# nunofachada/cl_ops

Hardware: AMD Instinct MI355X
Metric: Mkeys/s sorting 2^28 uint32 (satradix, 4-bit digits); achieved % of HBM roofline (higher is better)
Workload: dtype u32

## Files before the change

### cl_ops_amd/_hip.py

```python
import ctypes as C
import os

_HERE = os.path.dirname(os.path.abspath(__file__))
LIB_PATH = os.environ.get("CLO_HIP_LIBRARY") or os.path.join(_HERE, "lib", "libcl_ops_hip.so")

if not os.path.exists(LIB_PATH):
    raise ImportError(
        "cl_ops_amd: %s is missing. Build it with `python -c 'import __graft_entry__ as g; g.build()'` "
        "or `make -C cl_ops_amd/csrc` (needs hipcc). There is no fallback path." % LIB_PATH)

lib = C.CDLL(LIB_PATH, mode=C.RTLD_GLOBAL)

vp, sz, ci = C.c_void_p, C.c_size_t, C.c_int


class DeviceProps(C.Structure):
    _fields_ = [("name", C.c_char * 128), ("compute_units", ci), ("max_threads_per_block", ci),
                ("wavefront_size", ci), ("lds_bytes_per_block", sz), ("global_mem_bytes", sz),
                ("gcn_arch", C.c_char * 64)]


def _sig(name, restype, *argtypes):
    try:
        f = getattr(lib, name)
# ... 23 lines not shown
_sig("clo_hip_host_register", ci, vp, sz)
_sig("clo_hip_host_unregister", ci, vp)
_sig("clo_hip_stream_is_capturing", ci, vp)
_sig("clo_hip_graph_capture_begin", ci, vp)
_sig("clo_hip_graph_capture_end", ci, vp, C.POINTER(vp))
_sig("clo_hip_graph_launch", ci, vp, vp)
_sig("clo_hip_graph_destroy", ci, vp)
_sig("clo_hip_timing_enabled", ci)
_sig("clo_hip_event_create", ci, C.POINTER(vp))
_sig("clo_hip_event_destroy", ci, vp)
_sig("clo_hip_event_record", ci, vp, vp)
_sig("clo_hip_event_synchronize", ci, vp)
_sig("clo_hip_event_query", ci, vp)
_sig("clo_hip_env_refresh", None)
_sig("clo_hip_event_elapsed_ms", ci, vp, vp, C.POINTER(C.c_float))
_sig("clo_hip_stream_wait_event", ci, vp, vp)
_sig("clo_hip_error_string", C.c_char_p, ci)
_sig("clo_hip_scan_workspace_bytes", sz, sz, ci, ci)
_sig("clo_hip_scan_workspace_init", ci, vp, sz, vp)
_sig("clo_hip_scan_workspace_forget", ci, vp)
_sig("clo_hip_scan_workspace_set_epoch", ci, vp, C.c_uint, vp)
_sig("clo_hip_scan_exclusive", ci, vp, vp, sz, ci, ci, ci, vp, sz, vp)
_sig("clo_hip_scan_exclusive_carry", ci, vp, vp, sz, ci, ci, ci, vp, vp, vp, sz, vp)
_sig("clo_hip_scan_fp_workspace_bytes", sz, sz, ci)
_sig("clo_hip_scan_is_typed", ci, ci, ci)
_sig("clo_hip_scan_typed_workspace_bytes", sz, sz, ci)
_sig("clo_hip_scan_exclusive_typed", ci, vp, vp, sz, ci, ci, vp, sz, vp)
_sig("clo_hip_scan_exclusive_fp", ci, vp, vp, sz, ci, ci, vp, sz, vp)
_sig("clo_hip_reduce_sum", ci, vp, sz, ci, ci, vp, vp)
_sig("clo_hip_radix_workspace_bytes", sz, sz, ci, ci, ci)
_sig("clo_hip_radix_polls", ci, sz, ci, ci)
_sig("clo_hip_radix_sort", ci, vp, vp, vp, sz, ci, ci, ci, ci, ci, vp, sz, vp)
_sig("clo_hip_radix_takes_first_digits", ci, sz, ci, ci, ci)
_sig("clo_hip_radix_sort_fed", ci, vp, vp, vp, sz, ci, ci, ci, ci, ci, vp, vp, sz, vp)
_sig("clo_hip_radix_seg_workspace_bytes", sz, sz, ci, ci, ci)
_sig("clo_hip_radix_sort_segmented", ci, vp, vp, vp, sz, C.POINTER(sz), ci, C.POINTER(sz), C.POINTER(sz), C.POINTER(ci), ci,
     ci, ci, ci, ci, vp, sz, vp, C.POINTER(ci))
_sig("clo_hip_radix_sort_segmented2", ci, vp, vp, vp, vp, sz, C.POINTER(sz), ci, C.POINTER(sz), C.POINTER(sz), C.POINTER(ci), C.POINTER(ci), ci,
     ci, ci, ci, ci, vp, sz, vp, C.POINTER(ci))
_sig("clo_hip_msd_histogram", ci, vp, sz, ci, ci, ci, ci, vp, vp)
_sig("clo_hip_msd_partition", ci, vp, vp, sz, ci, ci, ci, ci, vp, vp, sz, vp)
_sig("clo_hip_msd_workspace_bytes", sz, sz, ci, ci)
_sig("clo_hip_bitonic_padded_numel", sz, sz)
_sig("clo_hip_bitonic_simple", ci, vp, sz, ci, ci, ci, ci, ci, ci, C.POINTER(ci), vp)
_sig("clo_hip_bitonic_tiled", ci, vp, sz, ci, ci, ci, ci, ci, ci, C.POINTER(ci), vp)
_sig("clo_hip_bitonic_any", ci, vp, sz, ci, ci, ci, ci, ci, ci, C.POINTER(ci), vp)
_sig("clo_hip_kernel_lds_bytes", sz, C.c_char_p, ci, ci)
_sig("clo_hip_bitonic_jit_create", ci, ci, ci, C.c_char_p, C.c_char_p, C.c_char_p, C.POINTER(vp), C.POINTER(C.c_char_p))
_sig("clo_hip_bitonic_jit_destroy", None, vp)
_sig("clo_hip_bitonic_jit_sort", ci, vp, vp, sz, ci, C.POINTER(ci), vp)
_sig("clo_hip_bitonic_jit_gselect", ci, vp, vp, vp, sz, vp)
_sig("clo_hip_check_status", ci, vp, vp)
_sig("clo_hip_rccl_unique_id", ci, vp)
_sig("clo_hip_rccl_comm_create", ci, C.POINTER(vp), vp, ci, ci)
_sig("clo_hip_rccl_comm_destroy", ci, vp)
_sig("clo_hip_rccl_comm_abort", ci, vp)
_sig("clo_hip_rccl_all_gather_u64", ci, vp, vp, vp, sz, vp)
_sig("clo_hip_rccl_all_to_all_v", ci, vp, ci, ci, vp, vp, vp, vp, vp, vp, vp)
_sig("clo_hip_set_launch_observer", ci, vp, vp)
_sig("clo_hip_radix_jit_create", ci, ci, ci, C.c_char_p, C.c_char_p, C.POINTER(vp), C.POINTER(C.c_char_p))
_sig("clo_hip_radix_jit_destroy", None, vp)
_sig("clo_hip_radix_jit_sort", ci, vp, vp, vp, vp, vp, sz, ci, vp, sz, vp)
_sig("clo_hip_timing_enable", ci, ci)
_sig("clo_hip_timing_reset", ci)
_sig("clo_hip_timing_read", ci, C.c_char_p, C.POINTER(C.c_uint), C.POINTER(C.c_float))

# ... 27 lines not shown
```

### cl_ops_amd/csrc/hip/clo_hip_internal.h

```cpp
#ifndef CLO_HIP_INTERNAL_H
#define CLO_HIP_INTERNAL_H

#include <stddef.h>
#include <stdint.h>

#include "clo_hip.h"

#define CLO_WS_STATUS_OFFSET 0
#define CLO_WS_EPOCH_WORD    2
#define CLO_WS_DONE_WORD     3
#define CLO_WS_TICKET_WORD   16
#define CLO_WS_MAX_PASSES    64
#define CLO_WS_HEADER_BYTES  512

struct clo_hip_env_t { unsigned max_spins; int radix_sweep; int r1_pools; int no_digits; int bitonic_merge2; };
const clo_hip_env_t* clo_hip_env();
int clo_radixw_preload();

inline bool clo_misaligned(const void* p, size_t align) { return ((uintptr_t) p & (align - 1)) != 0; }
inline bool clo_ws_misaligned(const void* ws) { return clo_misaligned(ws, CLO_HIP_WORKSPACE_ALIGN); }

#ifdef __HIPCC__
#include <hip/hip_runtime.h>

void clo_timing_begin(const char* label, hipStream_t s);
void clo_timing_end(hipStream_t s);
struct clo_timing_scope {
	hipStream_t s;
	clo_timing_scope(const char* label, hipStream_t stream) : s(stream) { clo_timing_begin(label, s); }
	~clo_timing_scope() { clo_timing_end(s); }
};

struct clo_keyx {
	unsigned long long sign, field;
	int kind;
};
template <typename E>
__device__ __forceinline__ E clo_keyx_fwd(E x, const clo_keyx& k) {
	if (k.kind == 1) return (E) (x ^ (E) k.sign);
	if (k.kind == 2) return (E) (x ^ ((x & (E) k.sign) ? (E) k.field : (E) k.sign));
	return x;
}
template <typename E>
__device__ __forceinline__ E clo_keyx_inv(E x, const clo_keyx& k) {
	if (k.kind == 1) return (E) (x ^ (E) k.sign);
	if (k.kind == 2) return (E) (x ^ ((x & (E) k.sign) ? (E) k.sign : (E) k.field));
	return x;
}
inline clo_keyx clo_keyx_make(int kind, int key_shift, int key_bits) {
	clo_keyx k = { 0, 0, 0 };
	if (kind == 1 || kind == 2) {
		k.kind = kind;
		k.sign = 1ull << (key_shift + key_bits - 1);
		k.field = (key_bits >= 64 ? ~0ull : ((1ull << key_bits) - 1ull)) << key_shift;
	}
	return k;
}

struct clo_kv_io {
	const void* keys_in;
	const unsigned* values_in;
	void* keys_out;
	unsigned* values_out;
};

size_t clo_radix4_workspace_bytes(size_t n, int elem_size, int digit_bits, int key_bits);
int clo_radix4_sort_kv(const clo_kv_io& io, void* pairs_a, void* pairs_b, size_t n, int key_size, int key_shift,
	int key_bits, int digit_bits, clo_keyx kx, void* ws, hipStream_t s);
size_t clo_radix4_partition_workspace_bytes(size_t n, int elem_size, int bits);
int clo_radix4_partition(const void* src, void* dst, size_t n, int elem_size, unsigned shift, int bits,
	unsigned long long* counts, void* ws, hipStream_t s);
int clo_radix4_sort(const void* src, void* dst, void* tmp, size_t n, int elem_size, int key_shift,
	int key_bits, int digit_bits, clo_keyx kx, const unsigned char* first_dig, void* ws, hipStream_t s);
int clo_radix4_takes_first_digits(size_t n, int elem_size, int digit_bits);
size_t clo_radix4_lds_bytes(int elem_size, int digit_bits);
int clo_radix1_applies(size_t n, int elem_size, int digit_bits);
size_t clo_radix1_workspace_bytes(size_t n, int elem_size, int key_bits);
int clo_radix1_sort(const void* src, void* dst, void* tmp, size_t n, int elem_size, int key_shift, int key_bits,
	clo_keyx kx, void* ws, unsigned* status, hipStream_t s);
int clo_bitonic_tiled_e1(void* data, size_t numel, int key_shift, int key_bits, int key_size, int key_kind, int descending, int* launches, hipStream_t s);
int clo_bitonic_tiled_e2(void* data, size_t numel, int key_shift, int key_bits, int key_size, int key_kind, int descending, int* launches, hipStream_t s);
int clo_bitonic_tiled_e4(void* data, size_t numel, int key_shift, int key_bits, int key_size, int key_kind, int descending, int* launches, hipStream_t s);
int clo_bitonic_tiled_e8(void* data, size_t numel, int key_shift, int key_bits, int key_size, int key_kind, int descending, int* launches, hipStream_t s);
size_t clo_radixw_lds_bytes(int digit_bits);
struct clo_radix_counters { unsigned* thist; unsigned* toff; unsigned* partial; unsigned* tinfo; unsigned tiles; bool big; };
int clo_radixw_launch_tilehist(const void* in, size_t n, int elem_size, int bits, unsigned shift, unsigned mask,
	const clo_radix_counters& c, clo_keyx kx, hipStream_t s);
int clo_radixw_launch_tilehist_kv(const void* keys, size_t n, int key_size, int bits, unsigned shift, unsigned mask,
	const clo_radix_counters& c, clo_keyx kx, hipStream_t s);
int clo_radixw_launch_tilehist_bytes(const unsigned char* dig, size_t n, int elem_size, int bits, unsigned mask,
	const clo_radix_counters& c, hipStream_t s);
int clo_radixw_launch_offsets(int bits, const clo_radix_counters& c, const unsigned** dbase, hipStream_t s);
size_t clo_radixw_partial_rows(size_t tiles);

#define CLO_SEG_MAX 256
struct clo_seg_tile { unsigned in_base, count_seg, out_base, seg_n; };
struct clo_seg_chunk { unsigned t0, tend, c_first, seg_last; };
struct clo_seg_pieces {
	unsigned n[CLO_SEG_MAX], in_base[CLO_SEG_MAX];
	unsigned short seg[CLO_SEG_MAX];
};
struct clo_seg_tables { const clo_seg_tile* tiles; const clo_seg_chunk* chunks; unsigned ntiles, nchunks, nseg; };
int clo_radixw_launch_tilehist_seg(const void* in, const void* in2, const clo_seg_tables& sg, int elem_size, int bits, unsigned shift, unsigned mask,
	const clo_radix_counters& c, hipStream_t s);
int clo_radixw_launch_tilehist_bytes_seg(const unsigned char* dig, const clo_seg_tables& sg, int elem_size, int bits, unsigned mask,
	const clo_radix_counters& c, hipStream_t s);
int clo_radixw_launch_offsets_seg(int bits, const clo_radix_counters& c, const clo_seg_tables& sg, const unsigned** dbase, hipStream_t s);
// ... 86 lines not shown
```

### cl_ops_amd/csrc/hip/clo_hip_radix.hip

```cpp
#include <hip/hip_runtime.h>

#include "clo_hip.h"
#include "clo_hip_internal.h"

namespace {

constexpr int HIST_THREADS = 256;
constexpr int HIST_ITEMS = 16;

template <typename E>
__global__ __launch_bounds__(HIST_THREADS)
void clo_msd_hist_kernel(const E* __restrict__ in, size_t n, unsigned shift, unsigned mask,
	unsigned long long* __restrict__ counts) {
	__shared__ unsigned h[HIST_THREADS / 64][8];
	const unsigned tid = threadIdx.x, wave = tid >> 6;
	if (tid < (HIST_THREADS / 64) * 8) (&h[0][0])[tid] = 0;
	__syncthreads();
	const size_t chunk = (size_t) HIST_THREADS * HIST_ITEMS;
	for (size_t base = (size_t) blockIdx.x * chunk; base < n; base += (size_t) gridDim.x * chunk) {
		#pragma unroll
		for (int i = 0; i < HIST_ITEMS; ++i) {
			const size_t idx = base + (size_t) i * HIST_THREADS + tid;
			if (idx < n) atomicAdd(&h[wave][(unsigned) (in[idx] >> shift) & mask & 7u], 1u);
		}
// ... 3 lines not shown
		unsigned s = 0;
		#pragma unroll
		for (int w = 0; w < HIST_THREADS / 64; ++w) s += h[w][tid];
		if (s) atomicAdd(&counts[tid], (unsigned long long) s);
	}
}

template <typename E>
int msd_hist_impl(const void* src, size_t n, unsigned shift, unsigned mask, uint64_t* counts, hipStream_t s) {
	unsigned blocks = (unsigned) ((n + HIST_THREADS * HIST_ITEMS - 1) / (HIST_THREADS * HIST_ITEMS));
	if (blocks > 2048) blocks = 2048;
	if (blocks == 0) blocks = 1;
	hipLaunchKernelGGL((clo_msd_hist_kernel<E>), dim3(blocks), dim3(HIST_THREADS), 0, s,
		(const E*) src, n, shift, mask, (unsigned long long*) counts);
	return (int) hipGetLastError();
}

}

extern "C" {

size_t clo_hip_radix_workspace_bytes(size_t numel, int elem_size, int key_bits, int digit_bits) {
	if (digit_bits < 1 || digit_bits > 8 || key_bits < 1) return 0;
	return clo_radix4_workspace_bytes(numel, elem_size, digit_bits, key_bits);
}

int clo_hip_radix_polls(size_t numel, int elem_size, int digit_bits) {
	return clo_radix1_applies(numel, elem_size, digit_bits) ? 1 : 0;
}

int clo_hip_radix_takes_first_digits(size_t numel, int elem_size, int key_kind, int digit_bits) {
	return key_kind == 0 ? clo_radix4_takes_first_digits(numel, elem_size, digit_bits) : 0;
}

int clo_hip_radix_sort(const void* src, void* dst, void* tmp, size_t numel,
	int elem_size, int key_shift, int key_bits, int key_kind, int digit_bits,
	void* workspace, size_t workspace_bytes, void* stream) {
	return clo_hip_radix_sort_fed(src, dst, tmp, numel, elem_size, key_shift, key_bits, key_kind, digit_bits, nullptr,
		workspace, workspace_bytes, stream);
}

int clo_hip_radix_sort_fed(const void* src, void* dst, void* tmp, size_t numel,
	int elem_size, int key_shift, int key_bits, int key_kind, int digit_bits, const unsigned char* first_digits,
	void* workspace, size_t workspace_bytes, void* stream) {

	if (numel == 0) return 0;
	if (!src || !dst || !tmp || !workspace || tmp == src || tmp == dst || clo_ws_misaligned(workspace)) return CLO_HIP_EARGS;
	if (key_bits < 1 || key_shift < 0 || key_shift + key_bits > 8 * elem_size) return CLO_HIP_EARGS;
	if (key_kind < 0 || key_kind > 2) return CLO_HIP_EARGS;
	if (key_kind == 2 && key_bits != 16 && key_bits != 32 && key_bits != 64) return CLO_HIP_EARGS;
	if (digit_bits < 1 || digit_bits > 8) return CLO_HIP_EUNSUPPORTED;
	if (numel > 0xffffffffull) return CLO_HIP_EARGS;
	if (workspace_bytes < clo_hip_radix_workspace_bytes(numel, elem_size, key_bits, digit_bits)) return CLO_HIP_EWORKSPACE;
	hipStream_t s = (hipStream_t) stream;
	const clo_keyx kx = clo_keyx_make(key_kind, key_shift, key_bits);
	return clo_radix4_sort(src, dst, tmp, numel, elem_size, key_shift, key_bits, digit_bits, kx, first_digits, workspace, s);
}

size_t clo_hip_radix_kv_workspace_bytes(size_t numel, int key_size, int key_bits, int digit_bits) {
	if (key_size != 1 && key_size != 2 && key_size != 4) return 0;
	return clo_hip_radix_workspace_bytes(numel, 8, key_bits, digit_bits);
}

int clo_hip_radix_sort_kv(const void* keys_in, const void* values_in, void* keys_out, void* values_out, void* pairs_a, void* pairs_b,
	size_t numel, int key_size, int key_shift, int key_bits, int key_kind, int digit_bits,
	void* workspace, size_t workspace_bytes, void* stream) {
// ... 104 lines not shown
```

### cl_ops_amd/csrc/hip/clo_hip_radix4.hip

```cpp
#include <hip/hip_runtime.h>

#include <cstdlib>
#include <type_traits>

#include "clo_hip.h"
#include "clo_hip_internal.h"
#include "clo_hip_radix_rank.h"

namespace {

template <int KB> struct kv_key;
template <> struct kv_key<1> { typedef uint8_t type; };
template <> struct kv_key<2> { typedef uint16_t type; };
template <> struct kv_key<4> { typedef uint32_t type; };

template <int KB, int ITEMS>
__device__ __forceinline__ void kv_load_pairs(const clo_kv_io& kv, size_t at, unsigned valid, bool aligned, uint64_t (&pair)[ITEMS]) {
	typedef typename kv_key<KB>::type K;
	const K* kp = reinterpret_cast<const K*>(kv.keys_in) + at;
	K k[ITEMS];
	unsigned v[ITEMS];
	if (valid == (unsigned) ITEMS) {
		load_blocked<K, ITEMS>(kp, k, aligned);
		if (kv.values_in) {
			load_blocked<unsigned, ITEMS>(kv.values_in + at, v, aligned);
		} else {
			#pragma unroll
			for (int i = 0; i < ITEMS; ++i) v[i] = (unsigned) at + (unsigned) i;
		}
	} else {
		#pragma unroll
		for (int i = 0; i < ITEMS; ++i) {
			k[i] = (unsigned) i < valid ? kp[i] : (K) 0;
			v[i] = (unsigned) i < valid ? (kv.values_in ? kv.values_in[at + i] : (unsigned) at + (unsigned) i) : 0u;
		}
	}
	#pragma unroll
	for (int i = 0; i < ITEMS; ++i) pair[i] = ((uint64_t) k[i] << 32) | v[i];
}

template <int KB>
__device__ __forceinline__ void kv_store_pair(const clo_kv_io& kv, unsigned gi, uint64_t e) {
	typedef typename kv_key<KB>::type K;
	if (kv.keys_out) reinterpret_cast<K*>(kv.keys_out)[gi] = (K) (e >> 32);
	kv.values_out[gi] = (unsigned) e;
}

template <typename E, int LB, int HB, bool BIG, bool DIG = false, bool SEG = false, int KV_IN = 0, int KV_OUT = 0>
__global__ __launch_bounds__((pair_shape<E, BIG>::THREADS), (pair_shape<E, BIG>::THREADS >= 1024 ? 8 : 6))
void clo_radix4_pair_kernel(const E* __restrict__ in, E* __restrict__ out, size_t n,
	unsigned shift, unsigned mask_lo, unsigned mask_hi,
	const unsigned* __restrict__ thist, const unsigned* __restrict__ toff, const unsigned* __restrict__ dbase,
	const unsigned* __restrict__ tinfo, int aligned,
	clo_keyx kx_in, clo_keyx kx_out, unsigned char* __restrict__ dig_out = nullptr, unsigned next_shift = 0,
	const clo_seg_tile* __restrict__ tdesc = nullptr, const E* __restrict__ in2 = nullptr, clo_kv_io kv = clo_kv_io()) {
	static_assert((KV_IN == 0 && KV_OUT == 0) || (sizeof(E) == 8 && !SEG), "key-value passes: 8-byte pairs, one array");

	constexpr int THREADS = pair_shape<E, BIG>::THREADS;
	constexpr int ITEMS = pair_shape<E, BIG>::ITEMS;
	constexpr int TILE = THREADS * ITEMS;
	constexpr int WAVES = THREADS / 64;
	constexpr int R2 = 1 << (LB + HB);
	constexpr int HMAX = pc_words<(LB > HB ? LB : HB)>::H;
	static_assert(R2 <= 256 && R2 <= THREADS, "one thread per combined digit, scanned by the first four waves");

	__shared__ __attribute__((aligned(16))) E s_stage[TILE];
	constexpr bool ALIAS = pair_shape<E, BIG>::ALIAS;
	__shared__ unsigned s_end[ALIAS ? 1 : THREADS * PC_END_STRIDE];
	__shared__ unsigned s_wtot[WAVES][HMAX];
	__shared__ __attribute__((aligned(16))) unsigned s_wbase[WAVES][HMAX];
	__shared__ unsigned s_delta[R2];
	__shared__ unsigned s_w4[4];

	const unsigned tid = threadIdx.x, lane = tid & 63u, wave = tid >> 6;
	const unsigned per_xcd = SEG ? (unsigned) ((n + 7) / 8) : (unsigned) ((n + (size_t) TILE * 8 - 1) / ((size_t) TILE * 8));
	const unsigned tile = (blockIdx.x & 7u) * per_xcd + (blockIdx.x >> 3);
	size_t base = (size_t) tile * TILE;
	unsigned count, n32;
	if constexpr (SEG) {
		if (tile >= (unsigned) n) return;
		const clo_seg_tile td = tdesc[tile];
		base = (size_t) td.in_base;
		count = td.count_seg & 0xffffu;
		n32 = td.seg_n;
		out += td.out_base;
		if constexpr (DIG) dig_out += td.out_base;
		dbase += (size_t) ((td.count_seg >> 16) & 0x7fffu) * R2;
		if (td.count_seg >> 31) in = in2;
	} else {
		if (base >= n) return;
		count = (n - base) < (size_t) TILE ? (unsigned) (n - base) : (unsigned) TILE;
		n32 = n > 0xffffffffull ? 0xffffffffu : (unsigned) n;
	}
	const bool full = count == (unsigned) TILE;
	const unsigned tbase = tid * ITEMS;
	const unsigned mask2 = (mask_hi << LB) | mask_lo;

	__builtin_amdgcn_s_setprio(3);
	unsigned h2 = 0, goff = 0;
	if (tid < (unsigned) R2) {
		h2 = thist[(size_t) tile * R2 + tid];
		goff = toff[(size_t) tile * R2 + tid];
		if (dbase) goff += dbase[tid];
	}
	E key[ITEMS];
	if constexpr (KV_IN != 0) {
		kv_load_pairs<KV_IN, ITEMS>(kv, base + tbase, full ? (unsigned) ITEMS : (count > tbase ? count - tbase : 0u), aligned != 0, key);
	} else if (full) {
		if constexpr (SEG) load_blocked_unaligned<E, ITEMS>(in + base + tbase, key);
		else load_blocked<E, ITEMS>(in + base + tbase, key, aligned != 0);
	} else {
		#pragma unroll
		for (int i = 0; i < ITEMS; ++i) key[i] = (tbase + i < count) ? in[base + tbase + i] : (E) 0;
	}
	__builtin_amdgcn_s_setprio(0);
	if (kx_in.kind) {
		#pragma unroll
		for (int i = 0; i < ITEMS; ++i) key[i] = clo_keyx_fwd<E>(key[i], kx_in);
	}
	{
		const unsigned incl2 = clo_wave_scan_inclusive<unsigned>(h2, lane);
		if (lane == 63 && wave < 4) s_w4[wave] = incl2;
		if (tid < (unsigned) R2) s_delta[tid] = goff - (incl2 - h2);
	}

	const bool single = tinfo[tile] != 0u;

	if (!single) {
		pc_local_split<E, LB, THREADS, ITEMS, HMAX, pc_no_mid, pc_no_counted, ALIAS>(key, shift, mask_lo, count, s_stage, s_end, s_wtot, s_wbase);
	} else {
		if (full) {
			constexpr int PER = ITEMS * (int) sizeof(E) >= 16 ? 16 / (int) sizeof(E) : ITEMS;
			typedef E vec16 __attribute__((ext_vector_type(PER)));
			#pragma unroll
			for (int k = 0; k < ITEMS / PER; ++k) {
				vec16 t;
				#pragma unroll
				for (int q = 0; q < PER; ++q) t[q] = key[k * PER + q];
				*reinterpret_cast<vec16*>(&s_stage[tbase + k * PER]) = t;
			}
		} else {
			#pragma unroll
			for (int i = 0; i < ITEMS; ++i) if (tbase + i < count) s_stage[tbase + i] = key[i];
		}
		clo_lds_barrier();
	}

	if (tid < (unsigned) R2) {
		unsigned before = 0;
		#pragma unroll
		for (unsigned w = 0; w < 4; ++w) if (w < wave) before += s_w4[w];
		s_delta[tid] -= before;
	}
	if (single) {
		__syncthreads();
	} else if (mask_hi != 0) {
		if (full) {
			constexpr int PER = ITEMS * (int) sizeof(E) >= 16 ? 16 / (int) sizeof(E) : ITEMS;
			typedef E vec16 __attribute__((ext_vector_type(PER)));
			#pragma unroll
			for (int k = 0; k < ITEMS / PER; ++k) {
				const vec16 t = *reinterpret_cast<const vec16*>(&s_stage[tbase + k * PER]);
				#pragma unroll
				for (int q = 0; q < PER; ++q) key[k * PER + q] = t[q];
			}
		} else {
			#pragma unroll
			for (int i = 0; i < ITEMS; ++i) if (tbase + i < count) key[i] = s_stage[tbase + i];
		}
		pc_local_split<E, HB, THREADS, ITEMS, HMAX, pc_no_mid, pc_no_counted, ALIAS>(key, shift + LB, mask_hi, count, s_stage, s_end, s_wtot, s_wbase);
	} else {
		__syncthreads();
	}

	constexpr int VEC = sizeof(E) >= 8 ? 1 : 4;
	typedef E vecE __attribute__((ext_vector_type(VEC)));
	typedef E vecE_u __attribute__((ext_vector_type(VEC), aligned(sizeof(E))));
	const bool dig_bytes = DIG && VEC == 4 && (next_shift & 7u) == 0u && next_shift < 8u * (unsigned) sizeof(E);
	const unsigned dig_b = next_shift >> 3;
	const unsigned dig_sel_lo = 0x0c0c0400u + dig_b * 0x0101u, dig_sel_hi = 0x04000c0cu + dig_b * 0x01010000u;
	const unsigned nbits2 = (unsigned) __builtin_popcount(mask2);
	const auto scatter = [&](auto kx_tag) {
		constexpr bool KX = decltype(kx_tag)::value;
		#pragma unroll
		for (int j = 0; j < ITEMS / VEC; ++j) {
			const unsigned p = (j * THREADS + tid) * VEC;
			if (full) {
				const vecE v = *reinterpret_cast<const vecE*>(&s_stage[p]);
				const unsigned d0 = pc_digit<E>(v[0], shift, mask2, nbits2), dl = pc_digit<E>(v[VEC - 1], shift, mask2, nbits2);
				const unsigned gi0 = p + s_delta[d0];
				if (d0 == dl && gi0 <= n32 - VEC) {
					vecE vo = v;
					if constexpr (KX) {
						#pragma unroll
						for (int k = 0; k < VEC; ++k) vo[k] = clo_keyx_inv<E>(v[k], kx_out);
					}
					if constexpr (KV_OUT != 0) kv_store_pair<KV_OUT>(kv, gi0, vo[0]);
					else *reinterpret_cast<vecE_u*>(&out[gi0]) = vo;
					if constexpr (DIG) {
						if constexpr (VEC == 4) {
							typedef unsigned u32_u __attribute__((aligned(1)));
							unsigned dg;
							if (dig_bytes)
								dg = __builtin_amdgcn_perm((unsigned) v[1], (unsigned) v[0], dig_sel_lo) | __builtin_amdgcn_perm((unsigned) v[3], (unsigned) v[2], dig_sel_hi);
							else
								dg = ((unsigned) (v[0] >> next_shift) & 255u) | (((unsigned) (v[1] >> next_shift) & 255u) << 8)
									| (((unsigned) (v[2] >> next_shift) & 255u) << 16) | ((unsigned) (v[3] >> next_shift) << 24);
							*reinterpret_cast<u32_u*>(dig_out + gi0) = dg;
						} else {
							dig_out[gi0] = (unsigned char) (v[0] >> next_shift);
						}
					}
				} else {
					#pragma unroll
// ... 81 lines not shown
	L.tinfo = L.partial + ((clo_radixw_partial_rows(L.tiles) * R2 * sizeof(unsigned) + 255) & ~(size_t) 255);
	L.total = L.tinfo + ((L.tiles * sizeof(unsigned) + 255) & ~(size_t) 255);
	L.dig = 0;
	if (digits && clo_radix_digit_stream(n, elem_size)) {
		L.dig = L.total;
		L.total += (n + 255) & ~(size_t) 255;
	}
	return L;
}

template <typename Layout>
clo_radix_counters rp_counters(void* ws, const Layout& L, size_t tiles) {
	char* w = (char*) ws;
	return { (unsigned*) (w + L.thist), (unsigned*) (w + L.toff), (unsigned*) (w + L.partial), (unsigned*) (w + L.tinfo), (unsigned) tiles, L.big };
}

struct rp_digits { unsigned shift, mask_lo, mask_hi, mask, next_shift; };

template <int LB, int HB>
rp_digits rp_pass_digits(int p, int key_shift, int key_bits) {
	constexpr int PB = LB + HB;
	const int rem = key_bits - p * PB;
	const int bits = rem < PB ? rem : PB;
	const int lo_bits = bits < LB ? bits : LB, hi_bits = bits - lo_bits;
	rp_digits d;
	d.shift = (unsigned) (key_shift + p * PB);
	d.mask_lo = (1u << lo_bits) - 1u;
	d.mask_hi = (1u << hi_bits) - 1u;
	d.mask = (d.mask_hi << LB) | d.mask_lo;
	d.next_shift = d.shift + PB;
	return d;
}

template <typename E, int LB, int HB, bool SEG = false, int KB = 0>
void rp_launch_pass(const clo_radix_counters& c, const rp_digits& d, const E* in, E* out, size_t n, const unsigned* dbase, int aligned,
	clo_keyx kx_in, clo_keyx kx_out, unsigned char* dig_out, hipStream_t s, const clo_seg_tile* tdesc = nullptr, const E* in2 = nullptr,
	bool kv_in = false, bool kv_out = false, const clo_kv_io& kv = clo_kv_io()) {
	const unsigned tiles = SEG ? (unsigned) n : c.tiles;
	const auto launch = [&](auto big, auto dig, auto kvi, auto kvo) {
		constexpr bool BIG = decltype(big)::value, DIG = decltype(dig)::value;
		hipLaunchKernelGGL((clo_radix4_pair_kernel<E, LB, HB, BIG, DIG, SEG, decltype(kvi)::value, decltype(kvo)::value>),
			dim3((tiles + 7u) / 8u * 8u), dim3(pair_shape<E, BIG>::THREADS), 0, s,
			in, out, n, d.shift, d.mask_lo, d.mask_hi, c.thist, c.toff, dbase, c.tinfo, aligned, kx_in, kx_out, dig_out, d.next_shift, tdesc, in2, kv);
	};
	const auto shape = [&](auto kvi, auto kvo) {
		constexpr bool BIG_OK = sizeof(E) >= 4, DIG_OK = BIG_OK && LB == 4 && HB == 4 && decltype(kvo)::value == 0;
		if constexpr (DIG_OK) {
			if (c.big && dig_out) { launch(std::true_type(), std::true_type(), kvi, kvo); return; }
		}
		if constexpr (BIG_OK) {
			if (c.big) { launch(std::true_type(), std::false_type(), kvi, kvo); return; }
		}
		launch(std::false_type(), std::false_type(), kvi, kvo);
	};
	typedef std::integral_constant<int, 0> plain;
	typedef std::integral_constant<int, KB> key;
	if (kv_in && kv_out) shape(key(), key());
	else if (kv_in) shape(key(), plain());
	else if (kv_out) shape(plain(), key());
	else shape(plain(), plain());
}

int kv_unpack(const uint64_t* pairs, const clo_kv_io& io, size_t n, int key_size, hipStream_t s);

template <typename E, int LB, int HB, int KB = 0>
int rp_sort_impl(const E* src, E* dst, E* tmp, size_t n, int key_shift, int key_bits, clo_keyx kx, const unsigned char* first_dig,
	const clo_kv_io& kv, void* ws, hipStream_t s) {
	constexpr int PB = LB + HB;
	const int passes = (key_bits + PB - 1) / PB;
	const rp_layout L = rp_make_layout(n, (int) sizeof(E), PB);
	const clo_radix_counters c = rp_counters(ws, L, L.tiles);
	const bool no_dig = clo_hip_env()->no_digits != 0;
	constexpr bool DIG_OK = LB == 4 && HB == 4 && sizeof(E) >= 4;
	unsigned char* dig = (DIG_OK && L.dig != 0 && passes > 1 && !no_dig) ? (unsigned char*) ws + L.dig : nullptr;
	const clo_keyx kx_none = { 0, 0, 0 };
	const bool split_after = KB != 0 && passes == 1 && (kv.keys_out == kv.keys_in || (const void*) kv.values_out == (const void*) kv.values_in);
	const bool kv_aligned = (uintptr_t) kv.keys_in % 16 == 0 && (uintptr_t) kv.values_in % 16 == 0;

	hipError_t e;

	const bool inplace_odd = (dst == src) && (passes % 2 == 1);
	const E* cur_in = src;
	for (int p = 0; p < passes; ++p) {
		E* cur_out;
		if (inplace_odd) cur_out = (p % 2 == 0) ? tmp : dst;
		else cur_out = ((passes - 1 - p) % 2 == 0) ? dst : tmp;
		const bool kv_in = KB != 0 && p == 0, kv_out = KB != 0 && p + 1 == passes && !split_after;
		const rp_digits d = rp_pass_digits<LB, HB>(p, key_shift, key_bits);
		{
			clo_timing_scope timing("radix_hist", s);
			const unsigned char* hist_bytes = (dig && p > 0) ? dig : ((DIG_OK && c.big && p == 0 && kx.kind == 0) ? first_dig : nullptr);
			const int st = kv_in ? clo_radixw_launch_tilehist_kv(kv.keys_in, n, KB, PB, d.shift, d.mask, c, kx, s)
				: hist_bytes ? clo_radixw_launch_tilehist_bytes(hist_bytes, n, (int) sizeof(E), PB, d.mask, c, s)
				: clo_radixw_launch_tilehist(cur_in, n, (int) sizeof(E), PB, d.shift, d.mask, c, p == 0 ? kx : kx_none, s);
			if (st != 0) return st;
		}
		const unsigned* dbase = nullptr;
		{
			clo_timing_scope timing("radix_offsets", s);
			const int st = clo_radixw_launch_offsets(PB, c, &dbase, s);
			if (st != 0) return st;
		}
		{
			clo_timing_scope timing("radix_pass", s);
			const int aligned = kv_in ? (int) kv_aligned : (int) ((uintptr_t) cur_in % 16 == 0);
			rp_launch_pass<E, LB, HB, false, KB>(c, d, cur_in, cur_out, n, dbase, aligned, p == 0 ? kx : kx_none, p + 1 == passes ? kx : kx_none,
				p + 1 < passes ? dig : nullptr, s, nullptr, nullptr, kv_in, kv_out, kv);
		}
		cur_in = cur_out;
	}
	e = hipGetLastError();
	if (e != hipSuccess) return (int) e;
	if (inplace_odd) {
		e = hipMemcpyAsync(dst, tmp, n * sizeof(E), hipMemcpyDeviceToDevice, s);
		if (e != hipSuccess) return (int) e;
	}
	if constexpr (KB != 0) {
		if (split_after) return kv_unpack(dst, kv, n, KB, s);
	}
	return 0;
}

template <typename E>
int rp_dispatch(const void* src, void* dst, void* tmp, size_t n, int key_shift, int key_bits, int digit_bits,
	clo_keyx kx, const unsigned char* first_dig, void* ws, hipStream_t s) {
	#define CLO_RP(LB, HB) return rp_sort_impl<E, LB, HB>((const E*) src, (E*) dst, (E*) tmp, n, key_shift, key_bits, kx, first_dig, clo_kv_io(), ws, s)
	switch (digit_bits) {
		case 1: CLO_RP(1, 1);
		case 2: CLO_RP(2, 2);
		case 3: CLO_RP(3, 3);
		case 4: CLO_RP(4, 4);
		case 5: CLO_RP(3, 2);
		case 6: CLO_RP(3, 3);
		case 7: CLO_RP(4, 3);
		case 8: CLO_RP(4, 4);
		default: return CLO_HIP_EUNSUPPORTED;
	}
	#undef CLO_RP
}

// ... 236 lines not shown
	return CLO_HIP_EUNSUPPORTED;
}

size_t clo_radix4_partition_workspace_bytes(size_t n, int elem_size, int bits) {
	return rp_make_layout(n, elem_size, bits <= 3 ? 2 * bits : bits, false).total;
}

int clo_radix4_partition(const void* src, void* dst, size_t n, int elem_size, unsigned shift, int bits,
	unsigned long long* counts, void* ws, hipStream_t s) {
	#define CLO_R4P(E, B, LB, HB) return r4_partition_impl<E, B, LB, HB>((const E*) src, (E*) dst, n, shift, counts, ws, s)
	if (elem_size == 4) {
		if (bits == 1) CLO_R4P(uint32_t, 1, 1, 1);
		if (bits == 2) CLO_R4P(uint32_t, 2, 2, 2);
		if (bits == 3) CLO_R4P(uint32_t, 3, 3, 3);
		if (bits == 4) CLO_R4P(uint32_t, 4, 2, 2);
		if (bits == 5) CLO_R4P(uint32_t, 5, 3, 2);
		if (bits == 6) CLO_R4P(uint32_t, 6, 3, 3);
		if (bits == 7) CLO_R4P(uint32_t, 7, 4, 3);
		if (bits == 8) CLO_R4P(uint32_t, 8, 4, 4);
	} else if (elem_size == 8) {
		if (bits == 1) CLO_R4P(uint64_t, 1, 1, 1);
		if (bits == 2) CLO_R4P(uint64_t, 2, 2, 2);
		if (bits == 3) CLO_R4P(uint64_t, 3, 3, 3);
		if (bits == 4) CLO_R4P(uint64_t, 4, 2, 2);
		if (bits == 5) CLO_R4P(uint64_t, 5, 3, 2);
		if (bits == 6) CLO_R4P(uint64_t, 6, 3, 3);
		if (bits == 7) CLO_R4P(uint64_t, 7, 4, 3);
		if (bits == 8) CLO_R4P(uint64_t, 8, 4, 4);
	}
	#undef CLO_R4P
	return CLO_HIP_EUNSUPPORTED;
}

size_t clo_radix4_lds_bytes(int elem_size, int digit_bits) {
	const size_t threads = 512;
	const int half = digit_bits <= 4 ? digit_bits : (digit_bits + 1) / 2;
	const size_t hmax = half >= 4 ? 8 : (half == 3 ? 4 : (half == 2 ? 2 : 1));
	const size_t pass_bits = digit_bits <= 4 ? 2 * digit_bits : digit_bits;
	const size_t items = elem_size == 8 ? 8 : 16;
	return threads * items * (size_t) elem_size + threads * PC_END_STRIDE * sizeof(unsigned)
		+ (2 * (threads / 64) * hmax + ((size_t) 1 << pass_bits) + 4) * sizeof(unsigned);
}

int clo_radix4_takes_first_digits(size_t n, int elem_size, int digit_bits) {
	if (elem_size < 4 || (digit_bits != 4 && digit_bits != 8) || clo_hip_env()->no_digits) return 0;
	if (clo_radix1_applies(n, elem_size, digit_bits)) return 0;
	return clo_radix_big_tiles(n, elem_size) ? 1 : 0;
}

int clo_radix4_sort(const void* src, void* dst, void* tmp, size_t n, int elem_size, int key_shift,
	int key_bits, int digit_bits, clo_keyx kx, const unsigned char* first_dig, void* ws, hipStream_t s) {
	const size_t small_max = elem_size == 8 ? (size_t) small_big<uint64_t>::TILE : (size_t) small_big<uint32_t>::TILE;
	if (n <= small_max && digit_bits <= 4) {
		switch (elem_size) {
			case 1: return small_dispatch<uint8_t>(src, dst, n, key_shift, key_bits, digit_bits, kx, s);
			case 2: return small_dispatch<uint16_t>(src, dst, n, key_shift, key_bits, digit_bits, kx, s);
			case 4: return small_dispatch<uint32_t>(src, dst, n, key_shift, key_bits, digit_bits, kx, s);
			case 8: return small_dispatch<uint64_t>(src, dst, n, key_shift, key_bits, digit_bits, kx, s);
			default: return CLO_HIP_EUNSUPPORTED;
		}
	}
	if (clo_radix1_applies(n, elem_size, digit_bits))
		return clo_radix1_sort(src, dst, tmp, n, elem_size, key_shift, key_bits, kx,
			(char*) ws + r4_pair_workspace_bytes(n, elem_size, digit_bits), (unsigned*) ws, s);
	switch (elem_size) {
		case 1: return rp_dispatch<uint8_t>(src, dst, tmp, n, key_shift, key_bits, digit_bits, kx, first_dig, ws, s);
// ... 26 lines not shown
```

### cl_ops_amd/csrc/hip/clo_hip_runtime.hip

```cpp
#include <hip/hip_runtime.h>

#include <cstdio>
#include <cstring>
#include <mutex>
#include <string>
#include <vector>

#include "clo_hip.h"
#include "clo_hip_internal.h"

namespace {
struct timing_rec { std::string label; hipEvent_t e0, e1; };
std::mutex g_timing_mu;
std::vector<timing_rec> g_timing;
bool g_timing_on = false;
thread_local clo_hip_launch_observer g_observer = nullptr;
thread_local void* g_observer_user = nullptr;
}

void clo_timing_begin(const char* label, hipStream_t s) {
	if (g_observer) g_observer(g_observer_user, label, 0, (void*) s);
	if (!g_timing_on) return;
	std::lock_guard<std::mutex> lk(g_timing_mu);
	timing_rec r;
// ... 111 lines not shown
}
int clo_hip_free(void* dptr) { return dptr ? (int) hipFree(dptr) : 0; }

int clo_hip_memcpy_h2d_async(void* dst, const void* src, size_t bytes, void* stream) {
	return (int) hipMemcpyAsync(dst, src, bytes, hipMemcpyHostToDevice, (hipStream_t) stream);
}
int clo_hip_memcpy_d2h_async(void* dst, const void* src, size_t bytes, void* stream) {
	return (int) hipMemcpyAsync(dst, src, bytes, hipMemcpyDeviceToHost, (hipStream_t) stream);
}
int clo_hip_memcpy_d2d_async(void* dst, const void* src, size_t bytes, void* stream) {
	return (int) hipMemcpyAsync(dst, src, bytes, hipMemcpyDeviceToDevice, (hipStream_t) stream);
}
int clo_hip_memset_async(void* dst, int value, size_t bytes, void* stream) {
	return (int) hipMemsetAsync(dst, value, bytes, (hipStream_t) stream);
}

int clo_hip_host_register(void* host_ptr, size_t bytes) {
	if (!host_ptr || bytes == 0) return CLO_HIP_EARGS;
	return (int) hipHostRegister(host_ptr, bytes, hipHostRegisterDefault);
}
int clo_hip_host_unregister(void* host_ptr) { return host_ptr ? (int) hipHostUnregister(host_ptr) : 0; }

int clo_hip_event_create(void** event) {
	if (!event) return CLO_HIP_EARGS;
	hipEvent_t ev;
	hipError_t e = hipEventCreate(&ev);
	*event = (e == hipSuccess) ? (void*) ev : nullptr;
	return (int) e;
}
int clo_hip_event_destroy(void* event) { return event ? (int) hipEventDestroy((hipEvent_t) event) : 0; }
int clo_hip_event_record(void* event, void* stream) {
	return (int) hipEventRecord((hipEvent_t) event, (hipStream_t) stream);
}
static clo_hip_env_t g_env = { CLO_MAX_SPINS, 2, 0, 0, 1 };
static int g_env_read = 0;
void clo_hip_env_refresh(void) {
	clo_hip_env_t e = { CLO_MAX_SPINS, 2, 0, 0, 1 };
	if (const char* m = getenv("CLO_MAX_SPINS")) e.max_spins = (unsigned) strtoul(m, nullptr, 10);
	if (const char* m = getenv("CLO_RADIX_SWEEP")) e.radix_sweep = atoi(m) != 0 ? 1 : 0;
	if (const char* m = getenv("CLO_R1_POOLS")) e.r1_pools = atoi(m);
	e.no_digits = getenv("CLO_RADIX_NO_DIGITS") != nullptr;
	if (const char* m = getenv("CLO_BITONIC_MERGE2")) e.bitonic_merge2 = atoi(m);
	__atomic_store_n(&g_env.max_spins, e.max_spins, __ATOMIC_RELAXED);
	__atomic_store_n(&g_env.radix_sweep, e.radix_sweep, __ATOMIC_RELAXED);
	__atomic_store_n(&g_env.r1_pools, e.r1_pools, __ATOMIC_RELAXED);
	__atomic_store_n(&g_env.no_digits, e.no_digits, __ATOMIC_RELAXED);
	__atomic_store_n(&g_env.bitonic_merge2, e.bitonic_merge2, __ATOMIC_RELAXED);
	__atomic_store_n(&g_env_read, 1, __ATOMIC_RELEASE);
}
int clo_hip_event_synchronize(void* event) { return (int) hipEventSynchronize((hipEvent_t) event); }
int clo_hip_event_query(void* event) { return event ? (int) hipEventQuery((hipEvent_t) event) : CLO_HIP_EARGS; }
int clo_hip_event_elapsed_ms(void* start, void* stop, float* ms) {
	return ms ? (int) hipEventElapsedTime(ms, (hipEvent_t) start, (hipEvent_t) stop) : CLO_HIP_EARGS;
}
int clo_hip_stream_wait_event(void* stream, void* event) {
	return (int) hipStreamWaitEvent((hipStream_t) stream, (hipEvent_t) event, 0);
}

int clo_hip_graph_capture_begin(void* stream) {
	return (int) hipStreamBeginCapture((hipStream_t) stream, hipStreamCaptureModeThreadLocal);
}

int clo_hip_stream_is_capturing(void* stream) {
	hipStreamCaptureStatus st = hipStreamCaptureStatusNone;
	if (hipStreamIsCapturing((hipStream_t) stream, &st) != hipSuccess) { (void) hipGetLastError(); return 1; }
	return st != hipStreamCaptureStatusNone ? 1 : 0;
}

int clo_hip_graph_capture_end(void* stream, void** graph_exec) {
	if (!graph_exec) return CLO_HIP_EARGS;
	*graph_exec = nullptr;
	hipGraph_t graph = nullptr;
	hipError_t e = hipStreamEndCapture((hipStream_t) stream, &graph);
	if (e != hipSuccess) return (int) e;
	hipGraphExec_t exec = nullptr;
	e = hipGraphInstantiate(&exec, graph, nullptr, nullptr, 0);
	(void) hipGraphDestroy(graph);
	if (e != hipSuccess) return (int) e;
	*graph_exec = exec;
	return 0;
// ... 43 lines not shown
```

### include/clo_hip.h

```cpp
#ifndef CLO_HIP_H
#define CLO_HIP_H

#include <stddef.h>
#include <stdint.h>

#ifdef __cplusplus
extern "C" {
#endif

#define CLO_HIP_EARGS      (-1)
#define CLO_HIP_EUNSUPPORTED (-2)
#define CLO_HIP_EWORKSPACE (-3)
#define CLO_HIP_ETIMEOUT   (-4)
#define CLO_HIP_ENOTREADY  (-5)
#define CLO_HIP_ERCCL      (-100)

#define CLO_HIP_WORKSPACE_ALIGN 256


typedef struct {
	char name[128];
	int compute_units;
	int max_threads_per_block;
	int wavefront_size;
// ... 49 lines not shown
int clo_hip_scan_exclusive_carry(const void* data_in, void* data_out, size_t numel,
	int elem_size, int elem_signed, int sum_size,
	const uint64_t* carry_in_dev, uint64_t* carry_out_dev,
	void* workspace, size_t workspace_bytes, void* stream);
int clo_hip_scan_is_typed(int elem_type, int sum_type);
size_t clo_hip_scan_typed_workspace_bytes(size_t numel, int sum_type);
int clo_hip_scan_exclusive_typed(const void* data_in, void* data_out, size_t numel, int elem_type, int sum_type,
	void* workspace, size_t workspace_bytes, void* stream);
size_t clo_hip_scan_fp_workspace_bytes(size_t numel, int sum_size);
int clo_hip_scan_exclusive_fp(const void* data_in, void* data_out, size_t numel, int elem_type, int sum_size,
	void* workspace, size_t workspace_bytes, void* stream);
int clo_hip_reduce_sum(const void* data_in, size_t numel, int elem_size, int elem_signed,
	uint64_t* total_dev, void* stream);

size_t clo_hip_reduce_by_key_tile(int key_size, int value_size);
size_t clo_hip_reduce_by_key_workspace_bytes(size_t numel);
int clo_hip_reduce_by_key(const void* keys_in, const void* values_in, void* keys_out, void* aggr_out, uint64_t* num_runs_dev,
	size_t numel, int key_size, int value_type, int sum_type, int op,
	void* workspace, size_t workspace_bytes, void* stream);

size_t clo_hip_scan_by_key_tile(int key_size, int value_size);
size_t clo_hip_scan_by_key_workspace_bytes(size_t numel);
int clo_hip_scan_by_key(const void* keys_in, const void* values_in, void* out, size_t numel,
	int key_size, int value_type, int sum_type, int op, int inclusive,
	void* workspace, size_t workspace_bytes, void* stream);

int clo_hip_radix_preload(void);
size_t clo_hip_radix_workspace_bytes(size_t numel, int elem_size, int key_bits, int digit_bits);
int clo_hip_radix_polls(size_t numel, int elem_size, int digit_bits);
int clo_hip_radix_sort(const void* src, void* dst, void* tmp, size_t numel,
	int elem_size, int key_shift, int key_bits, int key_kind, int digit_bits,
	void* workspace, size_t workspace_bytes, void* stream);
int clo_hip_radix_takes_first_digits(size_t numel, int elem_size, int key_kind, int digit_bits);
int clo_hip_radix_sort_fed(const void* src, void* dst, void* tmp, size_t numel,
	int elem_size, int key_shift, int key_bits, int key_kind, int digit_bits, const unsigned char* first_digits,
	void* workspace, size_t workspace_bytes, void* stream);
size_t clo_hip_radix_kv_workspace_bytes(size_t numel, int key_size, int key_bits, int digit_bits);
int clo_hip_radix_sort_kv(const void* keys_in, const void* values_in, void* keys_out, void* values_out, void* pairs_a, void* pairs_b,
	size_t numel, int key_size, int key_shift, int key_bits, int key_kind, int digit_bits,
	void* workspace, size_t workspace_bytes, void* stream);
int clo_hip_radix_debug_stamps(void* buffer, size_t tiles);

size_t clo_hip_radix_seg_workspace_bytes(size_t numel, int nseg, int elem_size, int digit_bits);
int clo_hip_radix_sort_segmented(const void* src, void* a, void* b, size_t numel, const size_t* seg_counts, int nseg,
	const size_t* piece_counts, const size_t* piece_offsets, const int* piece_segment, int npieces,
	int elem_size, int key_shift, int key_bits, int digit_bits, void* workspace, size_t workspace_bytes, void* stream,
	int* result_in_b);
int clo_hip_radix_sort_segmented2(const void* src, const void* src2, void* a, void* b, size_t numel, const size_t* seg_counts, int nseg,
	const size_t* piece_counts, const size_t* piece_offsets, const int* piece_segment, const int* piece_source, int npieces,
	int elem_size, int key_shift, int key_bits, int digit_bits, void* workspace, size_t workspace_bytes, void* stream,
	int* result_in_b);

int clo_hip_msd_histogram(const void* src, size_t numel, int elem_size,
	int key_shift, int key_bits, int bucket_bits,
	uint64_t* counts_dev, void* stream);
int clo_hip_msd_partition(const void* src, void* dst, size_t numel, int elem_size,
	int key_shift, int key_bits, int bucket_bits, uint64_t* counts_dev,
	void* workspace, size_t workspace_bytes, void* stream);
size_t clo_hip_msd_workspace_bytes(size_t numel, int elem_size, int bucket_bits);

#define CLO_HIP_RCCL_ID_BYTES 128
int clo_hip_rccl_unique_id(void* id_out);
int clo_hip_rccl_comm_create(void** comm, const void* id_in, int rank, int world);
int clo_hip_rccl_comm_destroy(void* comm);
int clo_hip_rccl_comm_abort(void* comm);
int clo_hip_rccl_comm_async_error(void* comm);
// ... 54 lines not shown
```

Measured before the change: 113,100.

## Use unstable atomic LDS ranking for the first radix pass of plain key sorts

In an LSD radix sort of keys only, the first pass does not need to be stable, because the input order carries no meaning. For full tiles in that pass, the kernel now ranks keys with shared-memory atomicAdd on per-digit cursors and writes them straight into the LDS stage. This skips the multi-step stable local split. The shortcut applies only when no digit exceeds TILE/16 occurrences, which bounds atomic contention; otherwise the existing path runs. Setting CLO_RADIX_ORDERED_FIRST disables it, and a launch counter is exposed for checking that the path ran.

```diff
diff --git a/cl_ops_amd/_hip.py b/cl_ops_amd/_hip.py
--- a/cl_ops_amd/_hip.py
+++ b/cl_ops_amd/_hip.py
@@ -79,6 +79,7 @@
 _sig("clo_hip_radix_polls", ci, sz, ci, ci)
 _sig("clo_hip_radix_sort", ci, vp, vp, vp, sz, ci, ci, ci, ci, ci, vp, sz, vp)
 _sig("clo_hip_radix_takes_first_digits", ci, sz, ci, ci, ci)
+_sig("clo_hip_radix_unordered_launches", C.c_ulonglong)
 _sig("clo_hip_radix_sort_fed", ci, vp, vp, vp, sz, ci, ci, ci, ci, ci, vp, vp, sz, vp)
 _sig("clo_hip_radix_seg_workspace_bytes", sz, sz, ci, ci, ci)
 _sig("clo_hip_radix_sort_segmented", ci, vp, vp, vp, sz, C.POINTER(sz), ci, C.POINTER(sz), C.POINTER(sz), C.POINTER(ci), ci,
diff --git a/cl_ops_amd/csrc/hip/clo_hip_internal.h b/cl_ops_amd/csrc/hip/clo_hip_internal.h
--- a/cl_ops_amd/csrc/hip/clo_hip_internal.h
+++ b/cl_ops_amd/csrc/hip/clo_hip_internal.h
@@ -13,7 +13,7 @@
 #define CLO_WS_MAX_PASSES    64
 #define CLO_WS_HEADER_BYTES  512
 
-struct clo_hip_env_t { unsigned max_spins; int radix_sweep; int r1_pools; int no_digits; int bitonic_merge2; };
+struct clo_hip_env_t { unsigned max_spins; int radix_sweep; int r1_pools; int no_digits; int bitonic_merge2; int ordered_first; };
 const clo_hip_env_t* clo_hip_env();
 int clo_radixw_preload();
 
@@ -73,6 +73,7 @@
 int clo_radix4_sort(const void* src, void* dst, void* tmp, size_t n, int elem_size, int key_shift,
 	int key_bits, int digit_bits, clo_keyx kx, const unsigned char* first_dig, void* ws, hipStream_t s);
 int clo_radix4_takes_first_digits(size_t n, int elem_size, int digit_bits);
+unsigned long long clo_radix4_unordered_launches();
 size_t clo_radix4_lds_bytes(int elem_size, int digit_bits);
 int clo_radix1_applies(size_t n, int elem_size, int digit_bits);
 size_t clo_radix1_workspace_bytes(size_t n, int elem_size, int key_bits);
diff --git a/cl_ops_amd/csrc/hip/clo_hip_radix.hip b/cl_ops_amd/csrc/hip/clo_hip_radix.hip
--- a/cl_ops_amd/csrc/hip/clo_hip_radix.hip
+++ b/cl_ops_amd/csrc/hip/clo_hip_radix.hip
@@ -59,6 +59,8 @@
 int clo_hip_radix_takes_first_digits(size_t numel, int elem_size, int key_kind, int digit_bits) {
 	return key_kind == 0 ? clo_radix4_takes_first_digits(numel, elem_size, digit_bits) : 0;
 }
+
+unsigned long long clo_hip_radix_unordered_launches(void) { return clo_radix4_unordered_launches(); }
 
 int clo_hip_radix_sort(const void* src, void* dst, void* tmp, size_t numel,
 	int elem_size, int key_shift, int key_bits, int key_kind, int digit_bits,
diff --git a/cl_ops_amd/csrc/hip/clo_hip_radix4.hip b/cl_ops_amd/csrc/hip/clo_hip_radix4.hip
--- a/cl_ops_amd/csrc/hip/clo_hip_radix4.hip
+++ b/cl_ops_amd/csrc/hip/clo_hip_radix4.hip
@@ -46,7 +46,7 @@
 	kv.values_out[gi] = (unsigned) e;
 }
 
-template <typename E, int LB, int HB, bool BIG, bool DIG = false, bool SEG = false, int KV_IN = 0, int KV_OUT = 0>
+template <typename E, int LB, int HB, bool BIG, bool DIG = false, bool SEG = false, int KV_IN = 0, int KV_OUT = 0, bool UNORDERED = false>
 __global__ __launch_bounds__((pair_shape<E, BIG>::THREADS), (pair_shape<E, BIG>::THREADS >= 1024 ? 8 : 6))
 void clo_radix4_pair_kernel(const E* __restrict__ in, E* __restrict__ out, size_t n,
 	unsigned shift, unsigned mask_lo, unsigned mask_hi,
@@ -63,6 +63,8 @@
 	constexpr int R2 = 1 << (LB + HB);
 	constexpr int HMAX = pc_words<(LB > HB ? LB : HB)>::H;
 	static_assert(R2 <= 256 && R2 <= THREADS, "one thread per combined digit, scanned by the first four waves");
+	static_assert(!UNORDERED || (BIG && !SEG && KV_IN == 0 && KV_OUT == 0 && R2 == 256), "the plain sorts' first pass on big tiles");
+	constexpr unsigned UN_HEAVY = TILE / 16;
 
 	__shared__ __attribute__((aligned(16))) E s_stage[TILE];
 	constexpr bool ALIAS = pair_shape<E, BIG>::ALIAS;
@@ -71,6 +73,8 @@
 	__shared__ __attribute__((aligned(16))) unsigned s_wbase[WAVES][HMAX];
 	__shared__ unsigned s_delta[R2];
 	__shared__ unsigned s_w4[4];
+	__shared__ unsigned s_cur[UNORDERED ? R2 : 1];
+	__shared__ unsigned s_hv[UNORDERED ? 4 : 1];
 
 	const unsigned tid = threadIdx.x, lane = tid & 63u, wave = tid >> 6;
 	const unsigned per_xcd = SEG ? (unsigned) ((n + 7) / 8) : (unsigned) ((n + (size_t) TILE * 8 - 1) / ((size_t) TILE * 8));
@@ -97,36 +101,80 @@
 	const unsigned mask2 = (mask_hi << LB) | mask_lo;
 
 	__builtin_amdgcn_s_setprio(3);
-	unsigned h2 = 0, goff = 0;
+	unsigned h2 = 0, goff = 0, gbase = 0;
 	if (tid < (unsigned) R2) {
 		h2 = thist[(size_t) tile * R2 + tid];
 		goff = toff[(size_t) tile * R2 + tid];
-		if (dbase) goff += dbase[tid];
+		if (dbase) gbase = dbase[tid];
 	}
 	E key[ITEMS];
-	if constexpr (KV_IN != 0) {
-		kv_load_pairs<KV_IN, ITEMS>(kv, base + tbase, full ? (unsigned) ITEMS : (count > tbase ? count - tbase : 0u), aligned != 0, key);
-	} else if (full) {
-		if constexpr (SEG) load_blocked_unaligned<E, ITEMS>(in + base + tbase, key);
-		else load_blocked<E, ITEMS>(in + base + tbase, key, aligned != 0);
-	} else {
-		#pragma unroll
-		for (int i = 0; i < ITEMS; ++i) key[i] = (tbase + i < count) ? in[base + tbase + i] : (E) 0;
-	}
-	__builtin_amdgcn_s_setprio(0);
-	if (kx_in.kind) {
-		#pragma unroll
-		for (int i = 0; i < ITEMS; ++i) key[i] = clo_keyx_fwd<E>(key[i], kx_in);
-	}
-	{
+	const unsigned nbits2 = (unsigned) __builtin_popcount(mask2);
+
+	bool ranked = false, loaded = false;
+	if constexpr (UNORDERED) {
+		if (full) {
+			const unsigned incl2 = clo_wave_scan_inclusive<unsigned>(h2, lane);
+			goff += gbase;
+			if (tid < (unsigned) R2) {
+				if (lane == 63) s_w4[wave] = incl2;
+				s_delta[tid] = goff - (incl2 - h2);
+				const bool hv = __builtin_amdgcn_ballot_w64(h2 > UN_HEAVY) != 0ull;
+				if (lane == 0) s_hv[wave] = hv ? 1u : 0u;
+			}
+			load_blocked<E, ITEMS>(in + base + tbase, key, aligned != 0);
+			__builtin_amdgcn_s_setprio(0);
+			clo_lds_barrier();
+			ranked = (s_hv[0] | s_hv[1] | s_hv[2] | s_hv[3]) == 0u;
+			if (ranked) {
+				if (tid < (unsigned) R2) {
+					unsigned start = incl2 - h2;
+					#pragma unroll
+					for (unsigned w = 0; w < 4; ++w) if (w < wave) start += s_w4[w];
+					s_cur[tid] = start;
+					s_delta[tid] = goff - start;
+				}
+				clo_lds_barrier();
+			}
+			if (kx_in.kind) {
+				#pragma unroll
+				for (int i = 0; i < ITEMS; ++i) key[i] = clo_keyx_fwd<E>(key[i], kx_in);
+			}
+			if (ranked) {
+				#pragma unroll
+				for (int i = 0; i < ITEMS; ++i) {
+					const unsigned p = atomicAdd(&s_cur[pc_digit<E>(key[i], shift, mask2, nbits2)], 1u);
+					s_stage[p] = key[i];
+				}
+				__syncthreads();
+			}
+			loaded = true;
+		}
+	}
+	if (!loaded) {
+		if constexpr (KV_IN != 0) {
+			kv_load_pairs<KV_IN, ITEMS>(kv, base + tbase, full ? (unsigned) ITEMS : (count > tbase ? count - tbase : 0u), aligned != 0, key);
+		} else if (full) {
+			if constexpr (SEG) load_blocked_unaligned<E, ITEMS>(in + base + tbase, key);
+			else load_blocked<E, ITEMS>(in + base + tbase, key, aligned != 0);
+		} else {
+			#pragma unroll
+			for (int i = 0; i < ITEMS; ++i) key[i] = (tbase + i < count) ? in[base + tbase + i] : (E) 0;
+		}
+		__builtin_amdgcn_s_setprio(0);
+		if (kx_in.kind) {
+			#pragma unroll
+			for (int i = 0; i < ITEMS; ++i) key[i] = clo_keyx_fwd<E>(key[i], kx_in);
+		}
 		const unsigned incl2 = clo_wave_scan_inclusive<unsigned>(h2, lane);
 		if (lane == 63 && wave < 4) s_w4[wave] = incl2;
+		goff += gbase;
 		if (tid < (unsigned) R2) s_delta[tid] = goff - (incl2 - h2);
 	}
 
 	const bool single = tinfo[tile] != 0u;
 
-	if (!single) {
+	if (ranked) {
+	} else if (!single) {
 		pc_local_split<E, LB, THREADS, ITEMS, HMAX, pc_no_mid, pc_no_counted, ALIAS>(key, shift, mask_lo, count, s_stage, s_end, s_wtot, s_wbase);
 	} else {
 		if (full) {
@@ -146,13 +194,14 @@
 		clo_lds_barrier();
 	}
 
-	if (tid < (unsigned) R2) {
+	if (!ranked && tid < (unsigned) R2) {
 		unsigned before = 0;
 		#pragma unroll
 		for (unsigned w = 0; w < 4; ++w) if (w < wave) before += s_w4[w];
 		s_delta[tid] -= before;
 	}
-	if (single) {
+	if (ranked) {
+	} else if (single) {
 		__syncthreads();
 	} else if (mask_hi != 0) {
 		if (full) {
@@ -179,7 +228,6 @@
 	const bool dig_bytes = DIG && VEC == 4 && (next_shift & 7u) == 0u && next_shift < 8u * (unsigned) sizeof(E);
 	const unsigned dig_b = next_shift >> 3;
 	const unsigned dig_sel_lo = 0x0c0c0400u + dig_b * 0x0101u, dig_sel_hi = 0x04000c0cu + dig_b * 0x01010000u;
-	const unsigned nbits2 = (unsigned) __builtin_popcount(mask2);
 	const auto scatter = [&](auto kx_tag) {
 		constexpr bool KX = decltype(kx_tag)::value;
 		#pragma unroll
@@ -327,26 +375,37 @@
 	return d;
 }
 
+unsigned long long g_unordered_launches = 0;
+
 template <typename E, int LB, int HB, bool SEG = false, int KB = 0>
 void rp_launch_pass(const clo_radix_counters& c, const rp_digits& d, const E* in, E* out, size_t n, const unsigned* dbase, int aligned,
 	clo_keyx kx_in, clo_keyx kx_out, unsigned char* dig_out, hipStream_t s, const clo_seg_tile* tdesc = nullptr, const E* in2 = nullptr,
-	bool kv_in = false, bool kv_out = false, const clo_kv_io& kv = clo_kv_io()) {
+	bool kv_in = false, bool kv_out = false, const clo_kv_io& kv = clo_kv_io(), bool unordered = false) {
 	const unsigned tiles = SEG ? (unsigned) n : c.tiles;
-	const auto launch = [&](auto big, auto dig, auto kvi, auto kvo) {
+	const auto launch = [&](auto big, auto dig, auto kvi, auto kvo, auto un) {
 		constexpr bool BIG = decltype(big)::value, DIG = decltype(dig)::value;
-		hipLaunchKernelGGL((clo_radix4_pair_kernel<E, LB, HB, BIG, DIG, SEG, decltype(kvi)::value, decltype(kvo)::value>),
+		hipLaunchKernelGGL((clo_radix4_pair_kernel<E, LB, HB, BIG, DIG, SEG, decltype(kvi)::value, decltype(kvo)::value, decltype(un)::value>),
 			dim3((tiles + 7u) / 8u * 8u), dim3(pair_shape<E, BIG>::THREADS), 0, s,
 			in, out, n, d.shift, d.mask_lo, d.mask_hi, c.thist, c.toff, dbase, c.tinfo, aligned, kx_in, kx_out, dig_out, d.next_shift, tdesc, in2, kv);
 	};
 	const auto shape = [&](auto kvi, auto kvo) {
 		constexpr bool BIG_OK = sizeof(E) >= 4, DIG_OK = BIG_OK && LB == 4 && HB == 4 && decltype(kvo)::value == 0;
+		constexpr bool UN_OK = DIG_OK && !SEG && decltype(kvi)::value == 0;
+		if constexpr (UN_OK) {
+			if (c.big && unordered) {
+				if (dig_out) launch(std::true_type(), std::true_type(), kvi, kvo, std::true_type());
+				else launch(std::true_type(), std::false_type(), kvi, kvo, std::true_type());
+				__atomic_fetch_add(&g_unordered_launches, 1ull, __ATOMIC_RELAXED);
+				return;
+			}
+		}
 		if constexpr (DIG_OK) {
-			if (c.big && dig_out) { launch(std::true_type(), std::true_type(), kvi, kvo); return; }
+			if (c.big && dig_out) { launch(std::true_type(), std::true_type(), kvi, kvo, std::false_type()); return; }
 		}
 		if constexpr (BIG_OK) {
-			if (c.big) { launch(std::true_type(), std::false_type(), kvi, kvo); return; }
-		}
-		launch(std::false_type(), std::false_type(), kvi, kvo);
+			if (c.big) { launch(std::true_type(), std::false_type(), kvi, kvo, std::false_type()); return; }
+		}
+		launch(std::false_type(), std::false_type(), kvi, kvo, std::false_type());
 	};
 	typedef std::integral_constant<int, 0> plain;
 	typedef std::integral_constant<int, KB> key;
@@ -371,6 +430,8 @@
 	const clo_keyx kx_none = { 0, 0, 0 };
 	const bool split_after = KB != 0 && passes == 1 && (kv.keys_out == kv.keys_in || (const void*) kv.values_out == (const void*) kv.values_in);
 	const bool kv_aligned = (uintptr_t) kv.keys_in % 16 == 0 && (uintptr_t) kv.values_in % 16 == 0;
+	const bool unordered_first = KB == 0 && key_shift == 0 && key_bits == 8 * (int) sizeof(E) && passes > 1 && first_dig == nullptr
+		&& clo_hip_env()->ordered_first == 0;
 
 	hipError_t e;
 
@@ -400,7 +461,7 @@
 			clo_timing_scope timing("radix_pass", s);
 			const int aligned = kv_in ? (int) kv_aligned : (int) ((uintptr_t) cur_in % 16 == 0);
 			rp_launch_pass<E, LB, HB, false, KB>(c, d, cur_in, cur_out, n, dbase, aligned, p == 0 ? kx : kx_none, p + 1 == passes ? kx : kx_none,
-				p + 1 < passes ? dig : nullptr, s, nullptr, nullptr, kv_in, kv_out, kv);
+				p + 1 < passes ? dig : nullptr, s, nullptr, nullptr, kv_in, kv_out, kv, p == 0 && unordered_first);
 		}
 		cur_in = cur_out;
 	}
@@ -703,6 +764,8 @@
 	return CLO_HIP_EUNSUPPORTED;
 }
 
+unsigned long long clo_radix4_unordered_launches() { return __atomic_load_n(&g_unordered_launches, __ATOMIC_RELAXED); }
+
 size_t clo_radix4_lds_bytes(int elem_size, int digit_bits) {
 	const size_t threads = 512;
 	const int half = digit_bits <= 4 ? digit_bits : (digit_bits + 1) / 2;
diff --git a/cl_ops_amd/csrc/hip/clo_hip_runtime.hip b/cl_ops_amd/csrc/hip/clo_hip_runtime.hip
--- a/cl_ops_amd/csrc/hip/clo_hip_runtime.hip
+++ b/cl_ops_amd/csrc/hip/clo_hip_runtime.hip
@@ -167,20 +167,22 @@
 int clo_hip_event_record(void* event, void* stream) {
 	return (int) hipEventRecord((hipEvent_t) event, (hipStream_t) stream);
 }
-static clo_hip_env_t g_env = { CLO_MAX_SPINS, 2, 0, 0, 1 };
+static clo_hip_env_t g_env = { CLO_MAX_SPINS, 2, 0, 0, 1, 0 };
 static int g_env_read = 0;
 void clo_hip_env_refresh(void) {
-	clo_hip_env_t e = { CLO_MAX_SPINS, 2, 0, 0, 1 };
+	clo_hip_env_t e = { CLO_MAX_SPINS, 2, 0, 0, 1, 0 };
 	if (const char* m = getenv("CLO_MAX_SPINS")) e.max_spins = (unsigned) strtoul(m, nullptr, 10);
 	if (const char* m = getenv("CLO_RADIX_SWEEP")) e.radix_sweep = atoi(m) != 0 ? 1 : 0;
 	if (const char* m = getenv("CLO_R1_POOLS")) e.r1_pools = atoi(m);
 	e.no_digits = getenv("CLO_RADIX_NO_DIGITS") != nullptr;
 	if (const char* m = getenv("CLO_BITONIC_MERGE2")) e.bitonic_merge2 = atoi(m);
+	e.ordered_first = getenv("CLO_RADIX_ORDERED_FIRST") != nullptr;
 	__atomic_store_n(&g_env.max_spins, e.max_spins, __ATOMIC_RELAXED);
 	__atomic_store_n(&g_env.radix_sweep, e.radix_sweep, __ATOMIC_RELAXED);
 	__atomic_store_n(&g_env.r1_pools, e.r1_pools, __ATOMIC_RELAXED);
 	__atomic_store_n(&g_env.no_digits, e.no_digits, __ATOMIC_RELAXED);
 	__atomic_store_n(&g_env.bitonic_merge2, e.bitonic_merge2, __ATOMIC_RELAXED);
+	__atomic_store_n(&g_env.ordered_first, e.ordered_first, __ATOMIC_RELAXED);
 	__atomic_store_n(&g_env_read, 1, __ATOMIC_RELEASE);
 }
 int clo_hip_event_synchronize(void* event) { return (int) hipEventSynchronize((hipEvent_t) event); }
diff --git a/include/clo_hip.h b/include/clo_hip.h
--- a/include/clo_hip.h
+++ b/include/clo_hip.h
@@ -105,6 +105,7 @@
 	int elem_size, int key_shift, int key_bits, int key_kind, int digit_bits,
 	void* workspace, size_t workspace_bytes, void* stream);
 int clo_hip_radix_takes_first_digits(size_t numel, int elem_size, int key_kind, int digit_bits);
+unsigned long long clo_hip_radix_unordered_launches(void);
 int clo_hip_radix_sort_fed(const void* src, void* dst, void* tmp, size_t numel,
 	int elem_size, int key_shift, int key_bits, int key_kind, int digit_bits, const unsigned char* first_digits,
 	void* workspace, size_t workspace_bytes, void* stream);
```

New measurement: 107,400. 0.949x the previous value.
